# mklarqvist/libflagstats

Measured on AMD Instinct MI355X. Metric: Gflags/s + achieved HBM GB/s vs roofline, 8 GiB uint16, 1/2/4/8 MI355X, higher is better.
Workload: dtype u16

## Files before the change

libflagstats_amd/csrc/flagstat_segments.hip:

```cpp
#include <hip/hip_runtime.h>
#include <stdint.h>

#include <atomic>
#include <cstdio>
#include <cstring>
#include <memory>
#include <mutex>
#include <new>

#include "../../include/libflagstats_hip.h"
#include "flagstat_count_core.h"
#include "flagstat_engine.h"
#include "flagstat_segments.h"

namespace fsk {

constexpr int kSegDepth = 8;
constexpr int kSegRowVecs = 64;
constexpr int kSegUnitVecs = kSegWaveFlags / 8;

template <bool HAS_NEXT>
__device__ __forceinline__ void seg_step(Lane<kSegDepth>& s, uint4 (&v)[kUnroll], uint32_t blk, const uint4* __restrict__ cur,
                                         const uint4* __restrict__ next)
{
    uint32_t t8a = 0, t8b = 0, f8a = 0, f8b = 0, s8a = 0, s8b = 0;
#pragma unroll
    for (int half = 0; half < 2; ++half) {
        uint32_t t4a = 0, t4b = 0, f4a = 0, f4b = 0, s4a = 0, s4b = 0;
#pragma unroll
        for (int q = 0; q < 2; ++q) {
            uint32_t T[4], F[4], S[4];
#pragma unroll
            for (int k = 0; k < 2; ++k) {
                uint32_t L0, H0, L1, H1;
                const int uu = half * 4 + q * 2 + k;
                constexpr int RD = 6;
                __builtin_amdgcn_sched_barrier(0);
                split_out(v[uu], L0, H0, L1, H1);
                if (uu + RD < 8)
                    v[uu + RD] = load_vec<true>(cur + (uu + RD) * kSegRowVecs);
                else if constexpr (HAS_NEXT)
                    v[uu + RD - 8] = load_vec<true>(next + (uu + RD - 8) * kSegRowVecs);
                __builtin_amdgcn_sched_barrier(0);
                uint32_t qa, qb, ka, kb;
                front4(L0, H0, T[2 * k], qa, ka);
                front4(L1, H1, T[2 * k + 1], qb, kb);
                F[2 * k] = T[2 * k] & perm(0u, 0xFF00FF00u, qa);
                F[2 * k + 1] = T[2 * k + 1] & perm(0u, 0xFF00FF00u, qb);
                S[2 * k] = perm(0u, 0x84428140u, qa) & (ka | 0x3F3F3F3Fu);
                S[2 * k + 1] = perm(0u, 0x84428140u, qb) & (kb | 0x3F3F3F3Fu);
            }
            uint32_t t2a, t2b, f2a, f2b, s2a, s2b;
            csa(t2a, s.t1, s.t1, T[0], T[1]);
            csa(t2b, s.t1, s.t1, T[2], T[3]);
            csa(f2a, s.f1, s.f1, F[0], F[1]);
            csa(f2b, s.f1, s.f1, F[2], F[3]);
            csa(s2a, s.s1, s.s1, S[0], S[1]);
            csa(s2b, s.s1, s.s1, S[2], S[3]);
            csa(q ? t4b : t4a, s.t2, s.t2, t2a, t2b);
            csa(q ? f4b : f4a, s.f2, s.f2, f2a, f2b);
            csa(q ? s4b : s4a, s.s2, s.s2, s2a, s2b);
        }
        csa(half ? t8b : t8a, s.t4, s.t4, t4a, t4b);
        csa(half ? f8b : f8a, s.f4, s.f4, f4a, f4b);
        csa(half ? s8b : s8a, s.s4, s.s4, s4a, s4b);
    }
    uint32_t ct, cf, cs;
    csa(ct, s.t8, s.t8, t8a, t8b);
    csa(cf, s.f8, s.f8, f8a, f8b);
    csa(cs, s.s8, s.s8, s8a, s8b);
    chain_push<0, kSegDepth>(s, blk, ct, cf, cs);
}

template <bool HAS_NEXT>
__device__ __forceinline__ void seg_step_and_count(Lane<kSegDepth>& s, uint4 (&v)[kUnroll], uint32_t& blk, const uint4* cur,
                                                   const uint4* next)
{
    blk = __builtin_amdgcn_readfirstlane(blk);
    seg_step<HAS_NEXT>(s, v, blk, cur, next);
    ++blk;
    if (blk == (1u << kSegDepth) - 1u) {
        flush(s, (1u << kSegDepth) - 1u);
        blk = 0;
    }
}

__device__ __forceinline__ void count8(uint32_t (&acc)[kInternal], const uint4& x)
{
    const uint32_t L0 = perm(x.y, x.x, 0x06040200u), H0 = perm(x.y, x.x, 0x07050301u);
    const uint32_t L1 = perm(x.w, x.z, 0x06040200u), H1 = perm(x.w, x.z, 0x07050301u);
    uint32_t T0, T1, qa, qb, ka, kb;
    front4(L0, H0, T0, qa, ka);
    front4(L1, H1, T1, qb, kb);
    const uint32_t F0 = T0 & perm(0u, 0xFF00FF00u, qa), F1 = T1 & perm(0u, 0xFF00FF00u, qb);
    const uint32_t S0 = perm(0u, 0x84428140u, qa) & (ka | 0x3F3F3F3Fu), S1 = perm(0u, 0x84428140u, qb) & (kb | 0x3F3F3F3Fu);
#pragma unroll
    for (int c = 0; c < 8; ++c) {
        const uint32_t m = 0x01010101u << c;
        acc[c] += __builtin_popcount(T0 & m) + __builtin_popcount(T1 & m);
        acc[8 + c] += __builtin_popcount(F0 & m) + __builtin_popcount(F1 & m);
    }
#pragma unroll
    for (int c = 0; c < kInternal - 16; ++c) {
        const uint32_t m = 0x01010101u << (c < 3 ? c : c + 3);
        acc[16 + c] += __builtin_popcount(S0 & m) + __builtin_popcount(S1 & m);
    }
}

__device__ __forceinline__ uint4 mask_vec(uint4 x, uint64_t q, uint64_t b, uint64_t e)
{
    const uint32_t lk = b > q ? static_cast<uint32_t>(b - q < 8 ? b - q : 8) : 0u;
    const uint32_t hk = e > q ? static_cast<uint32_t>(e - q < 8 ? e - q : 8) : 0u;
    auto keep = [&](uint32_t k) { return k >= lk && k < hk; };
    x.x &= (keep(0) ? 0xFFFFu : 0u) | (keep(1) ? 0xFFFF0000u : 0u);
    x.y &= (keep(2) ? 0xFFFFu : 0u) | (keep(3) ? 0xFFFF0000u : 0u);
    x.z &= (keep(4) ? 0xFFFFu : 0u) | (keep(5) ? 0xFFFF0000u : 0u);
    x.w &= (keep(6) ? 0xFFFFu : 0u) | (keep(7) ? 0xFFFF0000u : 0u);
    return x;
}

__device__ __forceinline__ void count_piece(uint32_t (&acc)[kInternal], const uint4 (&v)[kUnroll], uint64_t w0, uint64_t b,
                                            uint64_t e, uint32_t lane)
{
#pragma unroll
    for (int r = 0; r < kUnroll; ++r) {
        const uint64_t r0 = w0 + static_cast<uint64_t>(r) * 512u;
        if (r0 + 512u <= b || r0 >= e) continue;
        if (r0 >= b && r0 + 512u <= e)
            count8(acc, v[r]);
        else
            count8(acc, mask_vec(v[r], r0 + 8u * lane, b, e));
    }
}

__device__ __forceinline__ uint64_t seg_slot_value(const uint32_t* tot, uint32_t t, int mode, uint64_t len)
{
    constexpr uint64_t kTOfSlot = 0x0652400187000300ull;
    const uint32_t slot = t & 15u;
    const bool fail = t >= 16;
    const int ti = static_cast<int>((kTOfSlot >> (4 * slot)) & 15u) - 1;
    uint64_t add = 0;
    if (ti >= 0) add = fail ? tot[8 + ti] : static_cast<uint64_t>(tot[ti]) - tot[8 + ti];
    if (slot == 10) add = fail ? tot[18] : tot[17];
    if (slot == 9 && fail) add = static_cast<uint64_t>(tot[16]) + tot[18];
    if (mode & 2) {
        if (slot == 0) add = fail ? tot[20] : tot[19];
        if (slot == 9 && !fail) add = len - (static_cast<uint64_t>(tot[16]) + tot[18]);
    }
    return add;
}

__device__ __forceinline__ uint64_t seg_pos(const uint64_t* __restrict__ off, uint64_t i, uint64_t base, uint64_t m, uint64_t lo0)
{
    uint64_t v = off[i];
    v = v < base ? base : v;
    v = v > base + m ? base + m : v;
    return v - base + lo0;
}

__device__ __forceinline__ uint64_t uniform64(uint64_t x)
{
    const uint32_t lo = __builtin_amdgcn_readfirstlane(static_cast<uint32_t>(x));
    const uint32_t hi = __builtin_amdgcn_readfirstlane(static_cast<uint32_t>(x >> 32));
    return (static_cast<uint64_t>(hi) << 32) | lo;
}

struct SegWalk {
    const uint64_t* off;
    uint64_t nseg, base, m, lo0;
    uint32_t lane;
    uint64_t wb;
    uint32_t wlo, whi;

    __device__ __forceinline__ void load_window(uint64_t first)
    {
        wb = first;
        const uint64_t i = first + lane;
        const uint64_t v = seg_pos(off, i <= nseg ? i : nseg, base, m, lo0);
        wlo = static_cast<uint32_t>(v);
        whi = static_cast<uint32_t>(v >> 32);
    }
    __device__ __forceinline__ void bounds(uint64_t s, uint64_t& sb, uint64_t& se)
    {
        if (s + 1 >= wb + 64) load_window(s);
        const int k = static_cast<int>(s - wb);
        sb = (static_cast<uint64_t>(static_cast<uint32_t>(__builtin_amdgcn_readlane(static_cast<int>(whi), k))) << 32) |
             static_cast<uint32_t>(__builtin_amdgcn_readlane(static_cast<int>(wlo), k));
        se = (static_cast<uint64_t>(static_cast<uint32_t>(__builtin_amdgcn_readlane(static_cast<int>(whi), k + 1))) << 32) |
             static_cast<uint32_t>(__builtin_amdgcn_readlane(static_cast<int>(wlo), k + 1));
    }
    __device__ __forceinline__ uint64_t first_segment(uint64_t p)
    {
        uint64_t lo = 1, hi = nseg + 1;
        while (lo < hi) {
            const uint64_t step = (hi - lo + 63) / 64;
            const uint64_t i = lo + lane * step;
            bool gt = true;
            if (i < hi) gt = seg_pos(off, i, base, m, lo0) > p;
            const uint64_t mask = __ballot(gt);
            if (mask == 0) {
                lo = lo + 63 * step + 1;
                continue;
            }
            const uint64_t f = static_cast<uint64_t>(__builtin_ctzll(mask));
            const uint64_t nhi = lo + f * step < hi ? lo + f * step : hi;
            lo = f ? lo + (f - 1) * step + 1 : lo;
            hi = nhi;
            lo = uniform64(lo);
            hi = uniform64(hi);
        }
        return lo - 1;
    }
};

__device__ __forceinline__ void seg_emit(Lane<kSegDepth>& st, uint32_t& blk, uint32_t* red, uint64_t* __restrict__ out, uint64_t s,
                                         uint64_t len, bool plain, int mode, uint32_t lane)
{
    if (blk) {
        flush(st, blk);
        blk = 0;
    }
    uint32_t w[kInternal];
#pragma unroll
    for (int c = 0; c < kInternal; ++c) {
        w[c] = wave_sum_lane63(st.acc[c]);
        st.acc[c] = 0;
    }
    if (lane == 63) {
#pragma unroll
        for (int c = 0; c < kInternal; ++c) red[c] = w[c];
    }
    __builtin_amdgcn_fence(__ATOMIC_RELEASE, "wavefront");
    __builtin_amdgcn_wave_barrier();
    __builtin_amdgcn_fence(__ATOMIC_ACQUIRE, "wavefront");
    if (lane < 32) {
        const uint64_t add = seg_slot_value(red, lane, mode, len);
        uint64_t* o = out + s * 32 + lane;
        if (plain)
            *o = add;
        else if (add)
            (void)__hip_atomic_fetch_add(o, add, __ATOMIC_RELAXED, __HIP_MEMORY_SCOPE_AGENT);
    }
    __builtin_amdgcn_wave_barrier();
}

__global__ __launch_bounds__(kThreads) void flagstat_segments(const uint4* __restrict__ a0, uint64_t lo0, uint64_t hi0, uint64_t base,
                                                              const uint64_t* __restrict__ off, uint64_t nseg,
                                                              uint64_t* __restrict__ out, int mode, uint64_t nunits,
                                                              uint32_t min_units)
{
    __shared__ uint32_t red_all[kThreads / 64][24];
    const uint32_t lane = threadIdx.x & 63u;
    const uint32_t wave = threadIdx.x >> 6;
    const uint64_t waves = static_cast<uint64_t>(gridDim.x) * (kThreads / 64);
    const uint64_t gw = static_cast<uint64_t>(blockIdx.x) * (kThreads / 64) + wave;
    const uint64_t u_begin = gw * nunits / waves, u_end = (gw + 1) * nunits / waves;
    const uint64_t p0 = u_begin * kSegWaveFlags > lo0 ? u_begin * kSegWaveFlags : lo0;
    const uint64_t E = u_end * kSegWaveFlags < hi0 ? u_end * kSegWaveFlags : hi0;
    if (p0 >= E) return;
    uint32_t* red = red_all[wave];

    SegWalk sw{off, nseg, base, hi0 - lo0, lo0, lane, 0, 0, 0};
    uint64_t s = sw.first_segment(p0);
    if (s >= nseg) return;
    sw.load_window(s);

    Lane<kSegDepth> st;
    lane_init(st);
    uint32_t blk = 0;
    bool open = false;
    uint64_t sb = 0, se = 0;
    auto emit = [&](uint64_t seg, uint64_t b_, uint64_t e_) {
        const uint64_t pb = b_ > p0 ? b_ : p0, pe = e_ < E ? e_ : E;
        seg_emit(st, blk, red, out, seg, pe - pb, (mode & 1) && b_ >= p0 && e_ <= E, mode, lane);
    };

    uint64_t u = p0 / kSegWaveFlags;
    while (s < nseg && u < u_end) {
        sw.bounds(s, sb, se);
        const uint64_t w0 = u * kSegWaveFlags;
        const uint64_t x = w0 > p0 ? w0 : p0;
        if (sb >= E) break;
        if (se <= sb || se <= x) {
            ++s;
            continue;
        }
        if (sb >= w0 + kSegWaveFlags) {
            u = sb / kSegWaveFlags;
            continue;
        }
        const uint64_t seg_e = se < E ? se : E;
        if (sb <= w0 && w0 >= lo0) {
            const uint64_t k = (seg_e - w0) / kSegWaveFlags;
            if (k >= min_units && k > 0) {
                const uint4* p = a0 + u * kSegUnitVecs + lane;
                uint4 v[kUnroll];
#pragma unroll
                for (int r = 0; r < 6; ++r) {
                    v[r] = load_vec<true>(p + r * kSegRowVecs);
                    __builtin_amdgcn_sched_barrier(0);
                }
                for (uint64_t i = 1; i < k; ++i) {
                    const uint4* pn = p + kSegUnitVecs;
                    seg_step_and_count<true>(st, v, blk, p, pn);
                    p = pn;
                }
                seg_step_and_count<false>(st, v, blk, p, nullptr);
                u += k;
                open = true;
                if (u * kSegWaveFlags >= se) {
                    emit(s, sb, se);
                    open = false;
                    ++s;
                }
                continue;
            }
        }
        uint4 v[kUnroll];
        const uint64_t j0 = u * kSegUnitVecs + lane;
        if (w0 >= lo0 && w0 + kSegWaveFlags <= hi0) {
#pragma unroll
            for (int r = 0; r < kUnroll; ++r) v[r] = load_vec<true>(a0 + j0 + r * kSegRowVecs);
        } else {
#pragma unroll
            for (int r = 0; r < kUnroll; ++r) v[r] = load_guarded(a0, j0 + r * kSegRowVecs, lo0, hi0);
        }
        const uint64_t w1 = w0 + kSegWaveFlags;
        uint64_t xx = x;
        for (;;) {
            const uint64_t b = sb > xx ? sb : xx, e = se < w1 ? se : w1;
            count_piece(st.acc, v, w0, b, e, lane);
            open = true;
            if (e < se) break;
            emit(s, sb, se);
            open = false;
            ++s;
            xx = e;
            bool more = false;
            while (s < nseg) {
                sw.bounds(s, sb, se);
                if (sb >= E) break;
                if (se <= sb || se <= xx) {
                    ++s;
                    continue;
                }
                more = sb < w1;
                break;
            }
            if (!more) break;
        }
        ++u;
    }
    if (open) emit(s, sb, se);
}

}

static std::atomic<uint32_t> g_seg_min_units{2};
static std::atomic<uint32_t> g_seg_blocks_per_cu{1};

extern "C" void fsk_segments_policy(uint32_t* min_units, uint32_t* blocks_per_cu)
{
    *min_units = g_seg_min_units.load();
    *blocks_per_cu = g_seg_blocks_per_cu.load();
}

extern "C" void fsk_set_segments_policy(uint32_t min_units, uint32_t blocks_per_cu)
{
    g_seg_min_units = min_units;
    g_seg_blocks_per_cu = blocks_per_cu < 1 ? 1 : (blocks_per_cu > 8 ? 8 : blocks_per_cu);
}

extern "C" hipError_t fsk_launch_segments(const uint16_t* d_chunk, uint64_t base, uint64_t m, const uint64_t* d_offsets, uint64_t nseg,
                                          uint64_t* d_out, int mode, uint32_t grid, hipStream_t stream)
{
    if (nseg == 0) return hipSuccess;
    if (d_out == nullptr || d_offsets == nullptr || grid == 0 || (m && d_chunk == nullptr)) return hipErrorInvalidValue;
    const uintptr_t addr = reinterpret_cast<uintptr_t>(d_chunk);
    if (addr & 1u) return hipErrorInvalidValue;
    if (mode & 1) {
        const hipError_t e = hipMemsetAsync(d_out, 0, nseg * 32 * sizeof(uint64_t), stream);
        if (e != hipSuccess) return e;
    }
    if (m == 0) return hipSuccess;
    const uintptr_t a0 = addr & ~static_cast<uintptr_t>(15);
    const uint64_t lo0 = (addr - a0) / 2, hi0 = lo0 + m;
    const uint64_t nunits = (hi0 + fsk::kSegWaveFlags - 1) / fsk::kSegWaveFlags;
    const uint64_t want = (nunits + 3) / 4;
    const uint32_t g = want < grid ? static_cast<uint32_t>(want) : grid;
    hipLaunchKernelGGL(fsk::flagstat_segments, dim3(g), dim3(fsk::kThreads), 0, stream, reinterpret_cast<const uint4*>(a0), lo0, hi0,
                       base, d_offsets, nseg, d_out, mode & 3, nunits, g_seg_min_units.load());
    return hipGetLastError();
}

using fsint::DeviceGuard;
using fsint::Engine;
using fsint::fail_hip;
using fsint::fail_text;

namespace {

#define SEG_TRY(expr)                                      \
    do {                                                   \
        hipError_t e_ = (expr);                            \
        if (e_ != hipSuccess) return fail_hip(#expr, e_);  \
    } while (0)

constexpr uint64_t kMaxSegments = (~0ull) / 256 - 1;

uint32_t seg_grid(const Engine& e) { return static_cast<uint32_t>(e.cus) * g_seg_blocks_per_cu.load(); }

int check_host_offsets(const uint64_t* offsets, uint64_t nseg, uint64_t n)
{
    char buf[192];
    for (uint64_t i = 0; i < nseg; ++i) {
        if (offsets[i + 1] < offsets[i]) {
            std::snprintf(buf, sizeof buf, "offsets must be non-decreasing: offsets[%llu] = %llu > offsets[%llu] = %llu",
                          static_cast<unsigned long long>(i), static_cast<unsigned long long>(offsets[i]),
                          static_cast<unsigned long long>(i + 1), static_cast<unsigned long long>(offsets[i + 1]));
            return fail_text(buf);
        }
    }
    if (offsets[nseg] > n) {
        std::snprintf(buf, sizeof buf, "offsets[nseg] = %llu exceeds the array's %llu flags",
                      static_cast<unsigned long long>(offsets[nseg]), static_cast<unsigned long long>(n));
        return fail_text(buf);
    }
    return 0;
}

int check_extent(const void* p, uint64_t bytes, const char* what)
{
    hipDeviceptr_t b = nullptr;
    size_t size = 0;
    if (hipMemGetAddressRange(&b, &size, const_cast<void*>(p)) != hipSuccess) {
        (void)hipGetLastError();
        return 0;
    }
    const uintptr_t end = reinterpret_cast<uintptr_t>(b) + size, at = reinterpret_cast<uintptr_t>(p);
    if (at < reinterpret_cast<uintptr_t>(b) || end - at < bytes) {
        char buf[192];
        std::snprintf(buf, sizeof buf, "%s (%p) is %llu bytes short of the %llu the call needs", what, p,
                      static_cast<unsigned long long>(bytes - (end > at ? end - at : 0)), static_cast<unsigned long long>(bytes));
        return fail_text(buf);
    }
    return 0;
}

struct SegBuffers {
    uint64_t* cnt = nullptr;
    uint64_t* off = nullptr;
    ~SegBuffers()
    {
        if (cnt) (void)hipFree(cnt);
        if (off) (void)hipFree(off);
    }
    int alloc(uint64_t nseg)
    {
        hipError_t e = hipMalloc(&cnt, nseg * 32 * sizeof(uint64_t));
        if (e != hipSuccess) {
            cnt = nullptr;
            (void)hipGetLastError();
            char buf[160];
            std::snprintf(buf, sizeof buf, "cannot allocate %llu bytes of device counters for %llu segments",
                          static_cast<unsigned long long>(nseg * 256), static_cast<unsigned long long>(nseg));
            return fail_text(buf);
        }
        e = hipMalloc(&off, (nseg + 1) * sizeof(uint64_t));
        if (e != hipSuccess) {
            off = nullptr;
            return fail_hip("hipMalloc(segment offsets)", e);
        }
        return 0;
    }
};

int host_args(const uint64_t* offsets, uint64_t nseg, const void* out)
{
    if (!offsets || !out) return fail_text("NULL offsets or out with nseg > 0");
    if (nseg > kMaxSegments) return fail_text("nseg is too large: its counters cannot be allocated");
    return 0;
}

struct HostRows {
    std::unique_ptr<uint64_t[]> p;
    uint64_t words = 0;
    int alloc(uint64_t nseg)
    {
        words = nseg * 32;
        p.reset(new (std::nothrow) uint64_t[words]);
        if (!p) {
            char buf[160];
            std::snprintf(buf, sizeof buf, "cannot allocate %llu bytes of host memory for the rows of %llu segments",
                          static_cast<unsigned long long>(words * 8), static_cast<unsigned long long>(nseg));
            return fail_text(buf);
        }
        return 0;
    }
};

void apply(uint64_t* out, const HostRows& got, int flags)
{
    if (flags & 1)
        std::memcpy(out, got.p.get(), got.words * sizeof(uint64_t));
    else
        for (uint64_t i = 0; i < got.words; ++i) out[i] += got.p[i];
}

}

extern "C" {

int FLAGSTATS_hip_device_u16_segments(const uint16_t* d_array, uint64_t n, const uint64_t* d_offsets, uint64_t nseg, uint64_t* d_out,
                                      int flags, void* stream)
{
    FS_ENTRY();
    if (flags & ~3) return fail_text("flags: bit 0 store, bit 1 superset; no other bits");
    if (nseg == 0) return 0;
    if (!d_offsets || !d_out) return fail_text("NULL d_offsets or d_out with nseg > 0");
    if (n && !d_array) return fail_text("NULL array with n > 0");
    if (nseg > kMaxSegments) return fail_text("nseg is too large for its counters to be a size");
    if (reinterpret_cast<uintptr_t>(d_array) & 1u) return fail_text("array must be 2-byte aligned");
    int dev_out = -1, dev = -1;
    bool plain = false;
    int rc = fsint::device_of_pointer(d_out, "d_out", &dev_out, &plain);
    if (rc) return rc;
    if (!plain) return fail_text("d_out must be device memory (the counters are added with device atomics)");
    rc = fsint::device_of_pointer(d_offsets, "d_offsets", &dev);
    if (rc) return rc;
    if (dev != dev_out) return fail_text("d_offsets and d_out live on different devices");
    if (n) {
        rc = fsint::device_of_pointer(d_array, "d_array", &dev);
        if (rc) return rc;
        if (dev != dev_out) return fail_text("d_array and d_out live on different devices");
    }
    Engine* e = fsint::engine_for_device(dev_out);
    if (!e) return -1;
    DeviceGuard guard(e->device);
    if (!guard.ok()) return -1;
    hipStream_t s = static_cast<hipStream_t>(stream);
    rc = fsint::check_stream_device(s, e->device);
    if (rc) return rc;
    if ((rc = check_extent(d_out, nseg * 32 * sizeof(uint64_t), "d_out")) || (rc = check_extent(d_offsets, (nseg + 1) * sizeof(uint64_t), "d_offsets")))
        return rc;
    if (n && (rc = check_extent(d_array, n * sizeof(uint16_t), "d_array"))) return rc;
    SEG_TRY(fsk_launch_segments(d_array, 0, n, d_offsets, nseg, d_out, flags & 3, seg_grid(*e), s));
    return 0;
}

int FLAGSTATS_hip_device_u16_segments_sync(const uint16_t* d_array, uint64_t n, const uint64_t* offsets, uint64_t nseg, uint64_t* out,
                                           int flags)
{
    FS_ENTRY();
    if (flags & ~3) return fail_text("flags: bit 0 store, bit 1 superset; no other bits");
    if (nseg == 0) return 0;
    int rc = host_args(offsets, nseg, out);
    if (rc) return rc;
    if (n && !d_array) return fail_text("NULL array with n > 0");
    if (reinterpret_cast<uintptr_t>(d_array) & 1u) return fail_text("array must be 2-byte aligned");
    Engine* ep = nullptr;
    if (n) {
        int dev = -1;
        rc = fsint::device_of_pointer(d_array, "d_array", &dev);
        if (rc) return rc;
        ep = fsint::engine_for_device(dev);
    } else {
        ep = fsint::default_engine();
    }
    if (!ep) return -1;
    Engine& e = *ep;
    std::lock_guard<std::mutex> lk(e.mu);
    if (fsint::engine_alive(e)) return -1;
    DeviceGuard guard(e.device);
    if (!guard.ok()) return -1;
    SegBuffers buf;
    HostRows got;
    if ((rc = buf.alloc(nseg)) || (rc = got.alloc(nseg))) return rc;
    if ((rc = check_host_offsets(offsets, nseg, n))) return rc;
    if (n && (rc = check_extent(d_array, n * sizeof(uint16_t), "d_array"))) return rc;
    hipStream_t s = e.stream[0];
    SEG_TRY(hipMemcpyAsync(buf.off, offsets, (nseg + 1) * sizeof(uint64_t), hipMemcpyHostToDevice, s));
    SEG_TRY(fsk_launch_segments(d_array, 0, n, buf.off, nseg, buf.cnt, 1 | (flags & 2), seg_grid(e), s));
    SEG_TRY(hipMemcpyAsync(got.p.get(), buf.cnt, got.words * sizeof(uint64_t), hipMemcpyDeviceToHost, s));
    SEG_TRY(hipStreamSynchronize(s));
    apply(out, got, flags);
    return 0;
}

int FLAGSTATS_hip_u16_x64_segments(const uint16_t* array, uint64_t n, const uint64_t* offsets, uint64_t nseg, uint64_t* out, int flags)
{
    FS_ENTRY();
    if (flags & ~3) return fail_text("flags: bit 0 store, bit 1 superset; no other bits");
    if (nseg == 0) return 0;
    int rc = host_args(offsets, nseg, out);
    if (rc) return rc;
    if (n && !array) return fail_text("NULL array with n > 0");
    Engine* ep = fsint::default_engine();
    if (!ep) return -1;
    Engine& e = *ep;
    std::lock_guard<std::mutex> lk(e.mu);
    if (fsint::engine_alive(e)) return -1;
    DeviceGuard guard(e.device);
    if (!guard.ok()) return -1;
    fsint::lz4_gpu_other_use(e);
    SegBuffers buf;
    HostRows got;
    if ((rc = buf.alloc(nseg)) || (rc = got.alloc(nseg))) return rc;
    if ((rc = check_host_offsets(offsets, nseg, n))) return rc;
    if ((rc = fsint::engine_second(e))) return rc;
    const uint64_t chunk = fsint::knobs().chunk_flags.load() < 8 ? 8 : fsint::knobs().chunk_flags.load();
    const uint64_t first = offsets[0], last = offsets[nseg];
    const int slots = last - first > chunk ? 2 : 1;
    for (int i = 0; i < slots; ++i)
        if ((rc = fsint::stage_reserve(e, i, last - first < chunk ? (last - first ? last - first : 1) : chunk))) return rc;
    hipStream_t s0 = e.stream[0];
    SEG_TRY(hipMemsetAsync(buf.cnt, 0, nseg * 32 * sizeof(uint64_t), s0));
    SEG_TRY(hipMemcpyAsync(buf.off, offsets, (nseg + 1) * sizeof(uint64_t), hipMemcpyHostToDevice, s0));
    if (slots == 2 && (rc = fsint::stream_wait_stream(e, e.stream[1], s0))) return rc;
    const uint32_t grid = seg_grid(e);
    const int mode = flags & 2;
    uint64_t k = 0;
    for (uint64_t pos = first; pos < last; pos += chunk, ++k) {
        const int sl = static_cast<int>(k % static_cast<uint64_t>(slots));
        const uint64_t c = last - pos < chunk ? last - pos : chunk;
        SEG_TRY(hipMemcpyAsync(e.stage[sl], array + pos, c * sizeof(uint16_t), hipMemcpyHostToDevice, e.stream[sl]));
        SEG_TRY(fsk_launch_segments(e.stage[sl], pos, c, buf.off, nseg, buf.cnt, mode, grid, e.stream[sl]));
    }
    if (slots == 2 && (rc = fsint::stream_wait_stream(e, s0, e.stream[1]))) return rc;
    SEG_TRY(hipMemcpyAsync(got.p.get(), buf.cnt, got.words * sizeof(uint64_t), hipMemcpyDeviceToHost, s0));
    SEG_TRY(hipStreamSynchronize(s0));
    if (slots == 2) SEG_TRY(hipStreamSynchronize(e.stream[1]));
    apply(out, got, flags);
    return 0;
}

}
```

Before: 3674.

## Count short segment pieces with bit-plane adders, dot products and permlane scatter reduction

Partial-segment counting no longer uses per-column popcounts on per-lane accumulators. Flags are first converted to byte-plane rows once per unit, then summed with a carry-save bit-plane adder sized to the piece length. Column counts come from udot8, and a permlane/DPP scatter reduction feeds wave-scope atomics into LDS. Chained counters are now flushed straight into the LDS reducer, and dense segment lists launch three times as many waves. The aim is to cut ALU and reduction cost when segments are many and short, at the price of more LDS atomics and a more intricate reduction path.

```diff
diff --git a/libflagstats_amd/csrc/flagstat_segments.hip b/libflagstats_amd/csrc/flagstat_segments.hip
--- a/libflagstats_amd/csrc/flagstat_segments.hip
+++ b/libflagstats_amd/csrc/flagstat_segments.hip
@@ -72,64 +72,199 @@
     chain_push<0, kSegDepth>(s, blk, ct, cf, cs);
 }
 
+__device__ __forceinline__ void chain_to_red(Lane<kSegDepth>& st, uint32_t pushed, uint32_t* red, uint32_t lane)
+{
+#pragma unroll
+    for (int c = 0; c < kInternal; ++c) st.acc[c] = 0;
+    flush(st, pushed);
+    uint32_t w[kInternal];
+#pragma unroll
+    for (int c = 0; c < kInternal; ++c) w[c] = wave_sum_lane63(st.acc[c]);
+    if (lane == 63) {
+#pragma unroll
+        for (int c = 0; c < kInternal; ++c)
+            (void)__hip_atomic_fetch_add(red + c, w[c], __ATOMIC_RELAXED, __HIP_MEMORY_SCOPE_WAVEFRONT);
+    }
+}
+
 template <bool HAS_NEXT>
 __device__ __forceinline__ void seg_step_and_count(Lane<kSegDepth>& s, uint4 (&v)[kUnroll], uint32_t& blk, const uint4* cur,
-                                                   const uint4* next)
+                                                   const uint4* next, uint32_t* red, uint32_t lane)
 {
     blk = __builtin_amdgcn_readfirstlane(blk);
     seg_step<HAS_NEXT>(s, v, blk, cur, next);
     ++blk;
     if (blk == (1u << kSegDepth) - 1u) {
-        flush(s, (1u << kSegDepth) - 1u);
+        chain_to_red(s, (1u << kSegDepth) - 1u, red, lane);
         blk = 0;
     }
 }
 
-__device__ __forceinline__ void count8(uint32_t (&acc)[kInternal], const uint4& x)
+struct RowBytes {
+    uint32_t t[2], f[2], s[2];
+};
+
+__device__ __forceinline__ void row_bytes(const uint4& x, RowBytes& o)
 {
     const uint32_t L0 = perm(x.y, x.x, 0x06040200u), H0 = perm(x.y, x.x, 0x07050301u);
     const uint32_t L1 = perm(x.w, x.z, 0x06040200u), H1 = perm(x.w, x.z, 0x07050301u);
-    uint32_t T0, T1, qa, qb, ka, kb;
-    front4(L0, H0, T0, qa, ka);
-    front4(L1, H1, T1, qb, kb);
-    const uint32_t F0 = T0 & perm(0u, 0xFF00FF00u, qa), F1 = T1 & perm(0u, 0xFF00FF00u, qb);
-    const uint32_t S0 = perm(0u, 0x84428140u, qa) & (ka | 0x3F3F3F3Fu), S1 = perm(0u, 0x84428140u, qb) & (kb | 0x3F3F3F3Fu);
-#pragma unroll
-    for (int c = 0; c < 8; ++c) {
-        const uint32_t m = 0x01010101u << c;
-        acc[c] += __builtin_popcount(T0 & m) + __builtin_popcount(T1 & m);
-        acc[8 + c] += __builtin_popcount(F0 & m) + __builtin_popcount(F1 & m);
-    }
-#pragma unroll
-    for (int c = 0; c < kInternal - 16; ++c) {
-        const uint32_t m = 0x01010101u << (c < 3 ? c : c + 3);
-        acc[16 + c] += __builtin_popcount(S0 & m) + __builtin_popcount(S1 & m);
-    }
-}
-
-__device__ __forceinline__ uint4 mask_vec(uint4 x, uint64_t q, uint64_t b, uint64_t e)
-{
-    const uint32_t lk = b > q ? static_cast<uint32_t>(b - q < 8 ? b - q : 8) : 0u;
-    const uint32_t hk = e > q ? static_cast<uint32_t>(e - q < 8 ? e - q : 8) : 0u;
-    auto keep = [&](uint32_t k) { return k >= lk && k < hk; };
-    x.x &= (keep(0) ? 0xFFFFu : 0u) | (keep(1) ? 0xFFFF0000u : 0u);
-    x.y &= (keep(2) ? 0xFFFFu : 0u) | (keep(3) ? 0xFFFF0000u : 0u);
-    x.z &= (keep(4) ? 0xFFFFu : 0u) | (keep(5) ? 0xFFFF0000u : 0u);
-    x.w &= (keep(6) ? 0xFFFFu : 0u) | (keep(7) ? 0xFFFF0000u : 0u);
+    uint32_t qa, qb, ka, kb;
+    front4(L0, H0, o.t[0], qa, ka);
+    front4(L1, H1, o.t[1], qb, kb);
+    o.f[0] = o.t[0] & perm(0u, 0xFF00FF00u, qa);
+    o.f[1] = o.t[1] & perm(0u, 0xFF00FF00u, qb);
+    o.s[0] = perm(0u, 0x84428140u, qa) & (ka | 0x3F3F3F3Fu);
+    o.s[1] = perm(0u, 0x84428140u, qb) & (kb | 0x3F3F3F3Fu);
+}
+
+template <int NP>
+__device__ __forceinline__ void plane_add(uint32_t (&p)[NP], uint32_t x0, uint32_t x1)
+{
+    uint32_t c;
+    csa(c, p[0], p[0], x0, x1);
+#pragma unroll
+    for (int i = 1; i < NP - 1; ++i) {
+        const uint32_t k = p[i] & c;
+        p[i] ^= c;
+        c = k;
+    }
+    p[NP - 1] |= c;
+}
+
+template <uint32_t W>
+__device__ __forceinline__ void plane_counts(uint32_t pt, uint32_t pf, uint32_t ps, uint32_t (&c)[kInternal])
+{
+    constexpr uint32_t lo = W * 0x01010101u, hi = W * 0x10101010u;
+#pragma unroll
+    for (int j = 0; j < 4; ++j) {
+        const uint32_t m = 0x11111111u << j;
+        const uint32_t at = pt & m, af = pf & m;
+        c[j] = __builtin_amdgcn_udot8(at, lo, c[j], false);
+        c[j + 4] = __builtin_amdgcn_udot8(at, hi, c[j + 4], false);
+        c[8 + j] = __builtin_amdgcn_udot8(af, lo, c[8 + j], false);
+        c[12 + j] = __builtin_amdgcn_udot8(af, hi, c[12 + j], false);
+    }
+    const uint32_t a0 = ps & 0x11111111u, a1 = ps & 0x22222222u, a2 = ps & 0x44444444u, a3 = ps & 0x88888888u;
+    c[16] = __builtin_amdgcn_udot8(a0, lo, c[16], false);
+    c[17] = __builtin_amdgcn_udot8(a1, lo, c[17], false);
+    c[18] = __builtin_amdgcn_udot8(a2, lo, c[18], false);
+    c[19] = __builtin_amdgcn_udot8(a2, hi, c[19], false);
+    c[20] = __builtin_amdgcn_udot8(a3, hi, c[20], false);
+}
+
+template <int CTRL>
+__device__ __forceinline__ uint32_t dpp_u32(uint32_t x)
+{
+    return static_cast<uint32_t>(__builtin_amdgcn_update_dpp(0, static_cast<int>(x), CTRL, 0xF, 0xF, false));
+}
+
+__device__ __forceinline__ uint32_t wave_sum_scatter11(const uint32_t (&v)[11], uint32_t lane)
+{
+    uint32_t u[6];
+#pragma unroll
+    for (int i = 0; i < 6; ++i) {
+        const auto r = __builtin_amdgcn_permlane32_swap(v[2 * i], 2 * i + 1 < 11 ? v[2 * i + 1] : 0u, false, false);
+        u[i] = r[0] + r[1];
+    }
+    uint32_t w[3];
+#pragma unroll
+    for (int i = 0; i < 3; ++i) {
+        const auto r = __builtin_amdgcn_permlane16_swap(u[2 * i], u[2 * i + 1], false, false);
+        w[i] = r[0] + r[1];
+    }
+    const bool b3 = lane & 8u, b2 = lane & 4u;
+    const uint32_t z0 = (b3 ? w[1] : w[0]) + dpp_u32<0x140>(b3 ? w[0] : w[1]);
+    const uint32_t z1 = (b3 ? 0u : w[2]) + dpp_u32<0x140>(b3 ? w[2] : 0u);
+    uint32_t x = (b2 ? z1 : z0) + dpp_u32<0x141>(b2 ? z0 : z1);
+    x += dpp_u32<0x4E>(x);
+    x += dpp_u32<0xB1>(x);
     return x;
 }
 
-__device__ __forceinline__ void count_piece(uint32_t (&acc)[kInternal], const uint4 (&v)[kUnroll], uint64_t w0, uint64_t b,
-                                            uint64_t e, uint32_t lane)
-{
+struct ScatterSlot {
+    bool active;
+    uint32_t lo, hi, sh_lo, sh_hi;
+};
+
+__device__ __forceinline__ ScatterSlot scatter_slot(uint32_t lane)
+{
+    const uint32_t i = ((lane >> 2) & 1u) << 3 | ((lane >> 3) & 1u) << 2 | ((lane >> 4) & 1u) << 1 | ((lane >> 5) & 1u);
+    ScatterSlot q;
+    q.active = (lane & 3u) == 0 && i < 11;
+    if (i < 8) {
+        q.lo = i;
+        q.hi = 8 + i;
+        q.sh_lo = q.sh_hi = i & 3u;
+    } else {
+        q.lo = 16 + 2 * (i - 8);
+        q.hi = 17 + 2 * (i - 8);
+        q.sh_lo = i == 8 ? 0u : (i == 9 ? 2u : 3u);
+        q.sh_hi = i == 8 ? 1u : (i == 9 ? 2u : 0u);
+    }
+    return q;
+}
+
+template <int NP>
+__device__ __forceinline__ void piece_counts(const RowBytes (&rb)[kUnroll], int ra, int rz, uint64_t ms, uint64_t me,
+                                             uint32_t (&c)[kInternal])
+{
+    uint32_t pt[NP] = {}, pf[NP] = {}, ps[NP] = {};
 #pragma unroll
     for (int r = 0; r < kUnroll; ++r) {
-        const uint64_t r0 = w0 + static_cast<uint64_t>(r) * 512u;
-        if (r0 + 512u <= b || r0 >= e) continue;
-        if (r0 >= b && r0 + 512u <= e)
-            count8(acc, v[r]);
-        else
-            count8(acc, mask_vec(v[r], r0 + 8u * lane, b, e));
+        if (r < ra || r > rz) continue;
+        uint64_t m = ~0ull;
+        if (r == ra) m = ms;
+        if (r == rz) m &= me;
+        const uint32_t m0 = static_cast<uint32_t>(m), m1 = static_cast<uint32_t>(m >> 32);
+        plane_add<NP>(pt, rb[r].t[0] & m0, rb[r].t[1] & m1);
+        plane_add<NP>(pf, rb[r].f[0] & m0, rb[r].f[1] & m1);
+        plane_add<NP>(ps, rb[r].s[0] & m0, rb[r].s[1] & m1);
+    }
+#pragma unroll
+    for (int i = 0; i < kInternal; ++i) c[i] = 0;
+    plane_counts<1>(pt[0], pf[0], ps[0], c);
+    plane_counts<2>(pt[1], pf[1], ps[1], c);
+    if constexpr (NP >= 3) plane_counts<4>(pt[2], pf[2], ps[2], c);
+    if constexpr (NP >= 4) plane_counts<8>(pt[3], pf[3], ps[3], c);
+    if constexpr (NP >= 5) {
+        plane_counts<8>(pt[4], pf[4], ps[4], c);
+        plane_counts<8>(pt[4], pf[4], ps[4], c);
+    }
+}
+
+__device__ __forceinline__ uint64_t bytes_from(int t)
+{
+    return (~0ull << (4 * t)) << (4 * t);
+}
+
+__device__ __forceinline__ void count_piece(uint32_t* red, const RowBytes (&rb)[kUnroll], uint64_t w0, uint64_t b, uint64_t e,
+                                            uint32_t lane, const ScatterSlot& q)
+{
+    const int lb = __builtin_amdgcn_readfirstlane(static_cast<int>(b - w0));
+    const int le = __builtin_amdgcn_readfirstlane(static_cast<int>(e - w0));
+    const int ra = lb >> 9, rz = (le - 1) >> 9, n = rz - ra + 1;
+    const int ds = lb - (ra * 512 + 8 * static_cast<int>(lane)), de = le - (rz * 512 + 8 * static_cast<int>(lane));
+    const uint64_t ms = bytes_from(ds < 0 ? 0 : (ds > 8 ? 8 : ds));
+    const uint64_t me = ~bytes_from(de < 0 ? 0 : (de > 8 ? 8 : de));
+    uint32_t c[kInternal];
+    if (n == 1)
+        piece_counts<2>(rb, ra, rz, ms, me, c);
+    else if (n <= 3)
+        piece_counts<3>(rb, ra, rz, ms, me, c);
+    else if (n <= 7)
+        piece_counts<4>(rb, ra, rz, ms, me, c);
+    else
+        piece_counts<5>(rb, ra, rz, ms, me, c);
+    uint32_t v[11];
+#pragma unroll
+    for (int i = 0; i < 8; ++i) v[i] = c[i] | (c[8 + i] << 16);
+    v[8] = c[16] | (c[17] << 16);
+    v[9] = c[18] | (c[19] << 16);
+    v[10] = c[20];
+    const uint32_t x = wave_sum_scatter11(v, lane);
+    if (q.active) {
+        (void)__hip_atomic_fetch_add(red + q.lo, (x & 0xFFFFu) >> q.sh_lo, __ATOMIC_RELAXED, __HIP_MEMORY_SCOPE_WAVEFRONT);
+        (void)__hip_atomic_fetch_add(red + q.hi, x >> (16 + q.sh_hi), __ATOMIC_RELAXED, __HIP_MEMORY_SCOPE_WAVEFRONT);
     }
 }
 
@@ -213,26 +348,17 @@
     }
 };
 
-__device__ __forceinline__ void seg_emit(Lane<kSegDepth>& st, uint32_t& blk, uint32_t* red, uint64_t* __restrict__ out, uint64_t s,
-                                         uint64_t len, bool plain, int mode, uint32_t lane)
-{
-    if (blk) {
-        flush(st, blk);
-        blk = 0;
-    }
-    uint32_t w[kInternal];
-#pragma unroll
-    for (int c = 0; c < kInternal; ++c) {
-        w[c] = wave_sum_lane63(st.acc[c]);
-        st.acc[c] = 0;
-    }
-    if (lane == 63) {
-#pragma unroll
-        for (int c = 0; c < kInternal; ++c) red[c] = w[c];
-    }
+__device__ __forceinline__ void wave_sync()
+{
     __builtin_amdgcn_fence(__ATOMIC_RELEASE, "wavefront");
     __builtin_amdgcn_wave_barrier();
     __builtin_amdgcn_fence(__ATOMIC_ACQUIRE, "wavefront");
+}
+
+__device__ __forceinline__ void seg_emit(uint32_t* red, uint64_t* __restrict__ out, uint64_t s, uint64_t len, bool plain, int mode,
+                                         uint32_t lane)
+{
+    wave_sync();
     if (lane < 32) {
         const uint64_t add = seg_slot_value(red, lane, mode, len);
         uint64_t* o = out + s * 32 + lane;
@@ -241,7 +367,9 @@
         else if (add)
             (void)__hip_atomic_fetch_add(o, add, __ATOMIC_RELAXED, __HIP_MEMORY_SCOPE_AGENT);
     }
-    __builtin_amdgcn_wave_barrier();
+    wave_sync();
+    if (lane < 22) red[lane] = 0;
+    wave_sync();
 }
 
 __global__ __launch_bounds__(kThreads) void flagstat_segments(const uint4* __restrict__ a0, uint64_t lo0, uint64_t hi0, uint64_t base,
@@ -251,10 +379,10 @@
 {
     __shared__ uint32_t red_all[kThreads / 64][24];
     const uint32_t lane = threadIdx.x & 63u;
-    const uint32_t wave = threadIdx.x >> 6;
+    const uint32_t wave = __builtin_amdgcn_readfirstlane(threadIdx.x >> 6);
     const uint64_t waves = static_cast<uint64_t>(gridDim.x) * (kThreads / 64);
     const uint64_t gw = static_cast<uint64_t>(blockIdx.x) * (kThreads / 64) + wave;
-    const uint64_t u_begin = gw * nunits / waves, u_end = (gw + 1) * nunits / waves;
+    const uint64_t u_begin = uniform64(gw * nunits / waves), u_end = uniform64((gw + 1) * nunits / waves);
     const uint64_t p0 = u_begin * kSegWaveFlags > lo0 ? u_begin * kSegWaveFlags : lo0;
     const uint64_t E = u_end * kSegWaveFlags < hi0 ? u_end * kSegWaveFlags : hi0;
     if (p0 >= E) return;
@@ -265,14 +393,14 @@
     if (s >= nseg) return;
     sw.load_window(s);
 
-    Lane<kSegDepth> st;
-    lane_init(st);
-    uint32_t blk = 0;
+    if (lane < 22) red[lane] = 0;
+    wave_sync();
+    const ScatterSlot q = scatter_slot(lane);
     bool open = false;
     uint64_t sb = 0, se = 0;
     auto emit = [&](uint64_t seg, uint64_t b_, uint64_t e_) {
         const uint64_t pb = b_ > p0 ? b_ : p0, pe = e_ < E ? e_ : E;
-        seg_emit(st, blk, red, out, seg, pe - pb, (mode & 1) && b_ >= p0 && e_ <= E, mode, lane);
+        seg_emit(red, out, seg, pe - pb, (mode & 1) && b_ >= p0 && e_ <= E, mode, lane);
     };
 
     uint64_t u = p0 / kSegWaveFlags;
@@ -293,6 +421,9 @@
         if (sb <= w0 && w0 >= lo0) {
             const uint64_t k = (seg_e - w0) / kSegWaveFlags;
             if (k >= min_units && k > 0) {
+                Lane<kSegDepth> st;
+                lane_init(st);
+                uint32_t blk = 0;
                 const uint4* p = a0 + u * kSegUnitVecs + lane;
                 uint4 v[kUnroll];
 #pragma unroll
@@ -302,10 +433,11 @@
                 }
                 for (uint64_t i = 1; i < k; ++i) {
                     const uint4* pn = p + kSegUnitVecs;
-                    seg_step_and_count<true>(st, v, blk, p, pn);
+                    seg_step_and_count<true>(st, v, blk, p, pn, red, lane);
                     p = pn;
                 }
-                seg_step_and_count<false>(st, v, blk, p, nullptr);
+                seg_step_and_count<false>(st, v, blk, p, nullptr, red, lane);
+                if (blk) chain_to_red(st, blk, red, lane);
                 u += k;
                 open = true;
                 if (u * kSegWaveFlags >= se) {
@@ -316,20 +448,25 @@
                 continue;
             }
         }
-        uint4 v[kUnroll];
-        const uint64_t j0 = u * kSegUnitVecs + lane;
-        if (w0 >= lo0 && w0 + kSegWaveFlags <= hi0) {
-#pragma unroll
-            for (int r = 0; r < kUnroll; ++r) v[r] = load_vec<true>(a0 + j0 + r * kSegRowVecs);
-        } else {
-#pragma unroll
-            for (int r = 0; r < kUnroll; ++r) v[r] = load_guarded(a0, j0 + r * kSegRowVecs, lo0, hi0);
+        RowBytes rb[kUnroll];
+        {
+            uint4 v[kUnroll];
+            const uint64_t j0 = u * kSegUnitVecs + lane;
+            if (w0 >= lo0 && w0 + kSegWaveFlags <= hi0) {
+#pragma unroll
+                for (int r = 0; r < kUnroll; ++r) v[r] = load_vec<true>(a0 + j0 + r * kSegRowVecs);
+            } else {
+#pragma unroll
+                for (int r = 0; r < kUnroll; ++r) v[r] = load_guarded(a0, j0 + r * kSegRowVecs, lo0, hi0);
+            }
+#pragma unroll
+            for (int r = 0; r < kUnroll; ++r) row_bytes(v[r], rb[r]);
         }
         const uint64_t w1 = w0 + kSegWaveFlags;
         uint64_t xx = x;
         for (;;) {
             const uint64_t b = sb > xx ? sb : xx, e = se < w1 ? se : w1;
-            count_piece(st.acc, v, w0, b, e, lane);
+            count_piece(red, rb, w0, b, e, lane, q);
             open = true;
             if (e < se) break;
             emit(s, sb, se);
@@ -408,7 +545,13 @@
 
 constexpr uint64_t kMaxSegments = (~0ull) / 256 - 1;
 
-uint32_t seg_grid(const Engine& e) { return static_cast<uint32_t>(e.cus) * g_seg_blocks_per_cu.load(); }
+constexpr uint32_t kSegDenseWaves = 3;
+
+uint32_t seg_grid(const Engine& e, uint64_t nseg, uint64_t span)
+{
+    const uint32_t g = static_cast<uint32_t>(e.cus) * g_seg_blocks_per_cu.load();
+    return nseg > span / (2 * fsk::kSegWaveFlags) ? g * kSegDenseWaves : g;
+}
 
 int check_host_offsets(const uint64_t* offsets, uint64_t nseg, uint64_t n)
 {
@@ -544,7 +687,7 @@
     if ((rc = check_extent(d_out, nseg * 32 * sizeof(uint64_t), "d_out")) || (rc = check_extent(d_offsets, (nseg + 1) * sizeof(uint64_t), "d_offsets")))
         return rc;
     if (n && (rc = check_extent(d_array, n * sizeof(uint16_t), "d_array"))) return rc;
-    SEG_TRY(fsk_launch_segments(d_array, 0, n, d_offsets, nseg, d_out, flags & 3, seg_grid(*e), s));
+    SEG_TRY(fsk_launch_segments(d_array, 0, n, d_offsets, nseg, d_out, flags & 3, seg_grid(*e, nseg, n), s));
     return 0;
 }
 
@@ -580,7 +723,8 @@
     if (n && (rc = check_extent(d_array, n * sizeof(uint16_t), "d_array"))) return rc;
     hipStream_t s = e.stream[0];
     SEG_TRY(hipMemcpyAsync(buf.off, offsets, (nseg + 1) * sizeof(uint64_t), hipMemcpyHostToDevice, s));
-    SEG_TRY(fsk_launch_segments(d_array, 0, n, buf.off, nseg, buf.cnt, 1 | (flags & 2), seg_grid(e), s));
+    const uint32_t grid = seg_grid(e, nseg, offsets[nseg] - offsets[0]);
+    SEG_TRY(fsk_launch_segments(d_array, 0, n, buf.off, nseg, buf.cnt, 1 | (flags & 2), grid, s));
     SEG_TRY(hipMemcpyAsync(got.p.get(), buf.cnt, got.words * sizeof(uint64_t), hipMemcpyDeviceToHost, s));
     SEG_TRY(hipStreamSynchronize(s));
     apply(out, got, flags);
@@ -617,7 +761,7 @@
     SEG_TRY(hipMemsetAsync(buf.cnt, 0, nseg * 32 * sizeof(uint64_t), s0));
     SEG_TRY(hipMemcpyAsync(buf.off, offsets, (nseg + 1) * sizeof(uint64_t), hipMemcpyHostToDevice, s0));
     if (slots == 2 && (rc = fsint::stream_wait_stream(e, e.stream[1], s0))) return rc;
-    const uint32_t grid = seg_grid(e);
+    const uint32_t grid = seg_grid(e, nseg, last - first);
     const int mode = flags & 2;
     uint64_t k = 0;
     for (uint64_t pos = first; pos < last; pos += chunk, ++k) {
```

Result: no change. 3675 (median of 6 runs) (+0.0%).
